# SamArgt/AudioSourceSep

Hardware: NVIDIA B200
Metric: glow_log_prob_samples_per_s (higher is better)
Workload: dtype bf16

## Files before the change

audiosourcesep_b200/csrc/nn_tc.cu:

```cuda
#include "nn_tc_shared.cuh"

namespace asep {

namespace {

constexpr int kBarBytes4 = 256;
constexpr int kSmemBytes4 = kARegionBytes + kStages * kStageBytes + kBiasBytes + kBarBytes4;

template <bool kBwd, bool kSaveMask, bool kF16>
__global__ void __launch_bounds__(kThreadsTC2, 1) k_nn_tc4(const TCParams prm) {
  extern __shared__ __align__(1024) uint8_t smem[];
  if ((smem_u32(smem) & 1023u) != 0u) __trap();
  constexpr int S = kStages;
  uint8_t* sA = smem;
  uint8_t* sB = smem + kARegionBytes;
  float* sBias = reinterpret_cast<float*>(smem + kARegionBytes + S * kStageBytes);
  uint64_t* bars = reinterpret_cast<uint64_t*>(smem + kARegionBytes + S * kStageBytes + kBiasBytes);
  const uint32_t full0 = smem_u32(&bars[0]), empty0 = smem_u32(&bars[S]);
  const uint32_t a1_ready = smem_u32(&bars[2 * S]), accfull0 = smem_u32(&bars[2 * S + 1]);
  const uint32_t accfree_h0 = smem_u32(&bars[2 * S + 3]), panel0 = smem_u32(&bars[2 * S + 4]);
  const uint32_t cons0 = smem_u32(&bars[2 * S + 12]);
  uint32_t* tmem_slot = reinterpret_cast<uint32_t*>(&bars[2 * S + 16]);

  const int warp = threadIdx.x >> 5, lane = threadIdx.x & 31;
  if (threadIdx.x == 0) {
    for (int i = 0; i < S; ++i) {
      mbar_init(full0 + 8 * i, 1);
      mbar_init(empty0 + 8 * i, 1);
    }
    mbar_init(a1_ready, 8);
    mbar_init(accfull0, 1);
    mbar_init(accfull0 + 8, 1);
    mbar_init(accfree_h0, 8);
    for (int i = 0; i < 8; ++i) mbar_init(panel0 + 8 * i, 8);
    for (int i = 0; i < 4; ++i) mbar_init(cons0 + 8 * i, 1);
    fence_barrier_init();
  }
  if (warp == 2) tmem_alloc(smem_u32(tmem_slot), kTmemCols);
  tc_fence_before();
  __syncthreads();
  tc_fence_after();
  const uint32_t tmem_base = *tmem_slot;
  const uint32_t img3_bytes = (uint32_t)prm.n3p * 128u;

  if (warp == 0) {
    if (lane == 0) {
      uint32_t stage = 0, phase = 0;
      const uint8_t* w1 = reinterpret_cast<const uint8_t*>(prm.wimg);
      const uint8_t* w2 = w1 + (size_t)2 * prm.k1_panels * kStageBytes;
      const uint8_t* w3 = w2 + (size_t)2 * kNumPanels * kStageBytes;
      auto push = [&](const uint8_t* src, uint32_t bytes) {
        mbar_wait(empty0 + 8 * stage, phase ^ 1);
        mbar_expect_tx(full0 + 8 * stage, bytes);
        bulk_g2s(smem_u32(sB + stage * kStageBytes), src, bytes, full0 + 8 * stage);
        if (++stage == (uint32_t)S) { stage = 0; phase ^= 1; }
      };
      for (int round = 0; round < prm.num_rounds; ++round) {
        for (int half = 1; half >= 0; --half)
          for (int kp = 0; kp < prm.k1_panels; ++kp) push(w1 + (size_t)(half * prm.k1_panels + kp) * kStageBytes, kStageBytes);
        for (int i = 0; i < 2 * kNumPanels; ++i) push(w2 + (size_t)i * kStageBytes, kStageBytes);
        for (int kp = 0; kp < kNumPanels; ++kp) push(w3 + (size_t)kp * img3_bytes, img3_bytes);
      }
    }
  } else if (warp == 1) {
    if (lane == 0) {
      uint32_t stage = 0, phase = 0;
      const uint32_t a_base = smem_u32(sA);
      constexpr uint32_t idesc256 = make_idesc(256);
      constexpr uint32_t idesc256h = kF16 ? make_idesc_f16(256) : make_idesc(256);
      const uint32_t idesc3 = kF16 ? make_idesc_f16(prm.n3p) : make_idesc(prm.n3p);
      auto kblock = [&](uint32_t d_tmem, int kp, int steps, uint32_t idesc, bool first) {
        mbar_wait(full0 + 8 * stage, phase);
        tc_fence_after();
        const uint64_t da = make_desc(a_base + kp * kPanelBytes);
        const uint64_t db = make_desc(smem_u32(sB + stage * kStageBytes));
        for (int k = 0; k < steps; ++k) umma_bf16(d_tmem, da + (uint64_t)(2 * k), db + (uint64_t)(2 * k), idesc, !(first && k == 0));
        umma_commit(empty0 + 8 * stage);
        if (++stage == (uint32_t)S) { stage = 0; phase ^= 1; }
      };
      const uint32_t h0 = tmem_base, h1 = tmem_base + 256u;
      for (int round = 0; round < prm.num_rounds; ++round) {
        mbar_wait(a1_ready, round & 1);
        tc_fence_after();
        for (int kp = 0; kp < prm.k1_panels; ++kp) kblock(h1, kp, min(4, prm.k1_steps - 4 * kp), idesc256, kp == 0);
        umma_commit(accfull0 + 8);
        if (round > 0) {
          mbar_wait(accfree_h0, (round - 1) & 1);
          tc_fence_after();
        }
        for (int kp = 0; kp < prm.k1_panels; ++kp) kblock(h0, kp, min(4, prm.k1_steps - 4 * kp), idesc256, kp == 0);
        umma_commit(accfull0);
        for (int p = 0; p < 4; ++p) mbar_wait(panel0 + 8 * p, 0);
        tc_fence_after();
        for (int kp = 0; kp < kNumPanels; ++kp) {
          if (kp >= 4) {
            mbar_wait(panel0 + 8 * kp, 0);
            tc_fence_after();
          }
          kblock(h0, kp, 4, idesc256h, kp == 0);
        }
        umma_commit(accfull0);
        for (int kp = 0; kp < kNumPanels; ++kp) {
          kblock(h1, kp, 4, idesc256h, kp == 0);
          if (kp < 4) umma_commit(cons0 + 8 * kp);
        }
        umma_commit(accfull0 + 8);
        for (int p = 0; p < 4; ++p) mbar_wait(panel0 + 8 * p, 1);
        tc_fence_after();
        for (int kp = 0; kp < kNumPanels; ++kp) {
          if (kp >= 4) {
            mbar_wait(panel0 + 8 * kp, 1);
            tc_fence_after();
          }
          kblock(h0, kp, 4, idesc3, kp == 0);
        }
        umma_commit(accfull0);
      }
    }
  } else {
    const int lq = warp & 3;
    const int ch = (warp - 2) >> 2;
    const int row = lq * 32 + lane;
    const int wtid = threadIdx.x - 64;
    const uint32_t t_lane = tmem_base + ((uint32_t)(lq * 32) << 16);
    uint8_t* stg = sA + kARegionBytes - ((kTileM * prm.n3p * 4 + 1023) & ~1023);
    const int k1_pad = prm.k1_steps * 16;
    float4 b1v = make_float4(0.f, 0.f, 0.f, 0.f), b2v = b1v;
    if constexpr (!kBwd) {
      if (wtid < kF / 4) {
        b1v = __ldg(reinterpret_cast<const float4*>(prm.bias1) + wtid);
        b2v = __ldg(reinterpret_cast<const float4*>(prm.bias2) + wtid);
        reinterpret_cast<float4*>(sBias)[wtid] = b1v;
      }
    }
    auto arrive_warp = [&](uint32_t bar) {
      __syncwarp();
      if (lane == 0) mbar_arrive(bar);
    };
    const int tb = ch == 0 ? 0 : 5, te = ch == 0 ? 5 : 9;
    auto row_coords = [&](int round, long long& p, bool& valid, int& h, int& w) {
      const long long tile = (long long)round * prm.tiles_per_cta_round + blockIdx.x;
      p = tile * kTileM + row;
      valid = p < prm.M;
      w = 0; h = 0;
      if (valid) {
        const uint32_t pu = (uint32_t)p, q = pu / (uint32_t)prm.W;
        w = (int)(pu - q * (uint32_t)prm.W);
        h = (int)(q % (uint32_t)prm.H);
      }
    };
    auto finish_a1 = [&]() {
      if (ch == 1)
        for (int k = 2 * 9 * prm.src_ch; k < k1_pad; k += 2)
          *reinterpret_cast<uint32_t*>(sA + a_offset(row, k)) = 0u;
      fence_proxy_async();
      arrive_warp(a1_ready);
    };
    auto build = [&](int round) {
      long long p; bool valid; int h, w;
      row_coords(round, p, valid, h, w);
      build_a1_taps<16>(sA, row, prm.src, p, valid, h, w, prm.H, prm.W, prm.src_stride, prm.src_off, prm.tap_sign, tb, te);
      finish_a1();
    };
    const bool prefetch_regs = prm.src_ch <= 8;
    float pre[40];
    auto prefetch_a1 = [&](int round) {
      long long p; bool valid; int h, w;
      row_coords(round, p, valid, h, w);
      switch (prm.src_ch) {
        case 1: a1_load<1>(pre, prm.src, p, valid, h, w, prm.H, prm.W, prm.src_stride, prm.src_off, prm.tap_sign, tb, te); break;
        case 2: a1_load<2>(pre, prm.src, p, valid, h, w, prm.H, prm.W, prm.src_stride, prm.src_off, prm.tap_sign, tb, te); break;
        case 8: a1_load<8>(pre, prm.src, p, valid, h, w, prm.H, prm.W, prm.src_stride, prm.src_off, prm.tap_sign, tb, te); break;
        default: a1_load<4>(pre, prm.src, p, valid, h, w, prm.H, prm.W, prm.src_stride, prm.src_off, prm.tap_sign, tb, te); break;
      }
    };
    auto store_a1 = [&]() {
      switch (prm.src_ch) {
        case 1: a1_store<1>(sA, row, pre, tb, te); break;
        case 2: a1_store<2>(sA, row, pre, tb, te); break;
        case 8: a1_store<8>(sA, row, pre, tb, te); break;
        default: a1_store<4>(sA, row, pre, tb, te); break;
      }
      finish_a1();
    };
    for (int round = 0; round < prm.num_rounds; ++round) {
      const long long tile = (long long)round * prm.tiles_per_cta_round + blockIdx.x;
      const long long p = tile * kTileM + row;
      const bool valid = p < prm.M;
      const bool stamp = prm.dbg_out != nullptr && blockIdx.x == 0 && wtid == 0;
      long long* ts = prm.dbg_out + (long long)round * 8;
      if (prefetch_regs) {
        if (round == 0) { prefetch_a1(0); store_a1(); }
      } else {
        build(round);
      }
      if (stamp) ts[0] = clock64();
      if (ch == 0) {
        const long long pn = p + 2ll * prm.tiles_per_cta_round * kTileM;
        if (pn < prm.M) asm volatile("prefetch.global.L2 [%0];" ::"l"(prm.src + pn * prm.src_stride));
      }
#pragma unroll 1
      for (int gemm = 0; gemm < 2; ++gemm) {
        uint32_t* mask = kBwd ? (gemm == 0 ? prm.mask2 : prm.mask1) : (gemm == 0 ? prm.mask1 : prm.mask2);
        __nv_bfloat16* dump = gemm == 0 ? prm.dump1 : prm.dump2;
        uint32_t mkl[4] = {0u, 0u, 0u, 0u}, mkh[4] = {0u, 0u, 0u, 0u};
        if constexpr (kBwd) {
          if (valid) {
            const uint4 m0 = __ldg(reinterpret_cast<const uint4*>(mask + p * (kF / 32) + ch * 8));
            const uint4 m1 = __ldg(reinterpret_cast<const uint4*>(mask + p * (kF / 32) + ch * 8) + 1);
            mkl[0] = m0.x; mkl[1] = m0.y; mkl[2] = m0.z; mkl[3] = m0.w; mkh[0] = m1.x; mkh[1] = m1.y; mkh[2] = m1.z; mkh[3] = m1.w;
          }
        }
        if (gemm == 0 && wtid == 0) bulk_wait_read_all();
        if (!kBwd || gemm == 0) named_bar_sync(1, kWorkers2);
#pragma unroll 1
        for (int hh = 0; hh < 2; ++hh) {
          const uint32_t par = hh == 0 ? (uint32_t)(round + gemm) & 1u : (uint32_t)gemm;
          mbar_wait(accfull0 + 8 * hh, par);
          tc_fence_after();
          uint32_t v[2][32];
          tmem_ld32(t_lane + (uint32_t)(hh * 256 + ch * 32), v[0]);
#pragma unroll
          for (int pp = 0; pp < 4; ++pp) {
            const int pn = 4 * hh + pp;
            const int j = 2 * pn + ch;
            tmem_ld_wait();
            if (pp + 1 < 4) tmem_ld32(t_lane + (uint32_t)(hh * 256 + (pp + 1) * 64 + ch * 32), v[(pp + 1) & 1]);
            uint32_t pk[16];
            if constexpr (!kBwd) {
              uint32_t bits = 0;
#pragma unroll
              for (int c4 = 0; c4 < 8; ++c4) {
                const float4 b4 = reinterpret_cast<const float4*>(sBias + j * 32)[c4];
                const float f0 = __uint_as_float(v[pp & 1][4 * c4 + 0]) + b4.x, f1 = __uint_as_float(v[pp & 1][4 * c4 + 1]) + b4.y;
                const float f2 = __uint_as_float(v[pp & 1][4 * c4 + 2]) + b4.z, f3 = __uint_as_float(v[pp & 1][4 * c4 + 3]) + b4.w;
                if constexpr (kSaveMask) {
                  bits |= (f0 > 0.f ? 1u : 0u) << (4 * c4) | (f1 > 0.f ? 1u : 0u) << (4 * c4 + 1) |
                          (f2 > 0.f ? 1u : 0u) << (4 * c4 + 2) | (f3 > 0.f ? 1u : 0u) << (4 * c4 + 3);
                }
                pk[2 * c4] = kF16 ? pack_relu_f16(f0, f1) : pack_relu_bf16(f0, f1);
                pk[2 * c4 + 1] = kF16 ? pack_relu_f16(f2, f3) : pack_relu_bf16(f2, f3);
              }
              if constexpr (kSaveMask) { if (hh) mkh[pp] = bits; else mkl[pp] = bits; }
            } else {
              const uint32_t bits = hh ? mkh[pp] : mkl[pp];
#pragma unroll
              for (int c2 = 0; c2 < 16; ++c2) {
                const float f0 = ((bits >> (2 * c2)) & 1u) ? __uint_as_float(v[pp & 1][2 * c2]) : 0.f;
                const float f1 = ((bits >> (2 * c2 + 1)) & 1u) ? __uint_as_float(v[pp & 1][2 * c2 + 1]) : 0.f;
                pk[c2] = pack_bf16(f0, f1);
              }
            }
            if (dump != nullptr && valid) {
#pragma unroll
              for (int c4 = 0; c4 < 4; ++c4) {
                uint32_t d[4];
#pragma unroll
                for (int q = 0; q < 4; ++q) {
                  if constexpr (!kF16) {
                    d[q] = pk[4 * c4 + q];
                  } else {
                    const float2 f = __half22float2(*reinterpret_cast<const __half2*>(&pk[4 * c4 + q]));
                    d[q] = pack_bf16(f.x, f.y);
                  }
                }
                *reinterpret_cast<uint4*>(dump + p * kF + j * 32 + c4 * 8) = make_uint4(d[0], d[1], d[2], d[3]);
              }
            }
            if (gemm == 1 && hh == 0) mbar_wait(cons0 + 8 * pn, round & 1);
            uint8_t* base = sA + pn * kPanelBytes + row * 128;
#pragma unroll
            for (int c4 = 0; c4 < 4; ++c4)
              *reinterpret_cast<uint4*>(base + (((ch * 4 + c4) ^ (row & 7)) << 4)) =
                  make_uint4(pk[4 * c4], pk[4 * c4 + 1], pk[4 * c4 + 2], pk[4 * c4 + 3]);
            if (hh == 0 ? pp == 3 : (pp & 1)) {
              fence_proxy_async();
              tc_fence_before();
              __syncwarp();
              if (lane == 0) {
                if (hh == 0) {
#pragma unroll
                  for (int q = 0; q < 4; ++q) mbar_arrive(panel0 + 8 * q);
                } else {
                  mbar_arrive(panel0 + 8 * (pn - 1));
                  mbar_arrive(panel0 + 8 * pn);
                }
              }
            }
          }
          if (gemm == 1 && hh == 0 && prefetch_regs && round + 1 < prm.num_rounds) prefetch_a1(round + 1);
        }
        if constexpr (kSaveMask) {
          if (valid) {
            uint4* mo = reinterpret_cast<uint4*>(mask + p * (kF / 32) + ch * 8);
            mo[0] = make_uint4(mkl[0], mkl[1], mkl[2], mkl[3]);
            mo[1] = make_uint4(mkh[0], mkh[1], mkh[2], mkh[3]);
          }
        }
        if constexpr (!kBwd) {
          named_bar_sync(1, kWorkers2);
          if (wtid < kF / 4) reinterpret_cast<float4*>(sBias)[wtid] = gemm == 0 ? b2v : b1v;
        }
        if (stamp) ts[1 + gemm] = clock64();
      }

      mbar_wait(accfull0, (uint32_t)(round + 2) & 1u);
      tc_fence_after();
      if (stamp) ts[3] = clock64();
      if (prefetch_regs && round + 1 < prm.num_rounds) store_a1();
      if (stamp) ts[4] = clock64();
      {
        uint8_t* stg_row = stg + (size_t)row * 16;
        for (int j = ch; j < prm.n3p / 16; j += 4) {
          uint32_t v[2][16];
          const bool two = j + 2 < prm.n3p / 16;
          tmem_ld16(t_lane + (uint32_t)(j * 16), v[0]);
          if (two) tmem_ld16(t_lane + (uint32_t)((j + 2) * 16), v[1]);
          tmem_ld_wait();
#pragma unroll
          for (int i = 0; i < 2; ++i) {
            if (i == 1 && !two) break;
#pragma unroll
            for (int c4 = 0; c4 < 4; ++c4)
              *reinterpret_cast<uint4*>(stg_row + (size_t)((j + 2 * i) * 4 + c4) * (kTileM * 16)) =
                  make_uint4(v[i][4 * c4], v[i][4 * c4 + 1], v[i][4 * c4 + 2], v[i][4 * c4 + 3]);
          }
        }
        tc_fence_before();
        arrive_warp(accfree_h0);
        fence_proxy_async();
        named_bar_sync(2, kWorkers2);
        if (wtid == 0) {
          if (tile * kTileM < prm.M)
            bulk_s2g(prm.out + tile * kTileM * prm.n3p, smem_u32(stg), (uint32_t)(kTileM * prm.n3p * 4));
        }
      }
      if (stamp) ts[5] = clock64();
    }
    if (wtid == 0) bulk_wait_all();
  }

  tc_fence_before();
  __syncthreads();
  if (warp == 2) tmem_dealloc(tmem_base, kTmemCols);
}

int g_num_sms = 0;

bool g_prof_on = false;
std::vector<TcProfToken> g_prof_recs, g_prof_pool;
double g_prof_flops = 0.0;
double g_next_flops = 0.0;


template <bool kBwd, bool kSaveMask, bool kF16>
void launch_tc4(const TCParams& prm, int grid, cudaStream_t s) {
  auto kern = k_nn_tc4<kBwd, kSaveMask, kF16>;
  static bool attr_set = false;
  if (!attr_set) {
    CUDA_CHECK(cudaFuncSetAttribute(kern, cudaFuncAttributeMaxDynamicSharedMemorySize, kSmemBytes4));
    attr_set = true;
  }
  const TcProfToken tok = nn_tc_prof_begin(s);
  kern<<<grid, kThreadsTC2, kSmemBytes4, s>>>(prm);
  ASEP_LAUNCH_CHECK();
  nn_tc_prof_end(tok, s, g_next_flops);
}

template <bool kBwd>
bool run_tc(TCParams prm, cudaStream_t s) {
  if (g_num_sms == 0) {
    int dev = 0;
    CUDA_CHECK(cudaGetDevice(&dev));
    CUDA_CHECK(cudaDeviceGetAttribute(&g_num_sms, cudaDevAttrMultiProcessorCount, dev));
  }
  {
    ASEP_CHECK(prm.k1_panels * kPanelBytes + ((kTileM * prm.n3p * 4 + 1023) & ~1023) <= kARegionBytes, ASEP_ERR_UNSUPPORTED,
               "coupling network shape outside the tcgen05 kernel (stage-1 panels %d, stage-3 columns %d)", prm.k1_panels, prm.n3p);
    ASEP_CHECK(prm.M < (1ll << 31), ASEP_ERR_UNSUPPORTED, "more than 2^31 pixels in one coupling-network launch");
    const long long tiles = (prm.M + kTileM - 1) / kTileM;
    const int grid = (int)std::min<long long>(tiles, g_num_sms);
    prm.tiles_per_cta_round = grid;
    prm.num_rounds = (int)((tiles + grid - 1) / grid);
    static long long* dbg = nullptr;
    static const bool timing = getenv("ASEP_TC_DBG_TIMING") != nullptr;
    if (timing) {
      if (!dbg) CUDA_CHECK(cudaMalloc(&dbg, 8 * 4096 * sizeof(long long)));
      ASEP_CHECK(prm.num_rounds <= 4096, ASEP_ERR_BAD_ARG, "too many rounds for the timing buffer");
      prm.dbg_out = dbg;
    }
    if constexpr (kBwd) {
      launch_tc4<true, false, false>(prm, grid, s);
    } else {
      const bool save = prm.mask1 != nullptr;
      if (prm.f16) { if (save) launch_tc4<false, true, true>(prm, grid, s); else launch_tc4<false, false, true>(prm, grid, s); }
      else { if (save) launch_tc4<false, true, false>(prm, grid, s); else launch_tc4<false, false, false>(prm, grid, s); }
    }
    if (timing) {
      CUDA_CHECK(cudaStreamSynchronize(s));
      std::vector<long long> h((size_t)8 * prm.num_rounds);
      CUDA_CHECK(cudaMemcpy(h.data(), dbg, h.size() * sizeof(long long), cudaMemcpyDeviceToHost));
      double d[6] = {0};
      const int r0 = prm.num_rounds > 2 ? 1 : 0, r1 = prm.num_rounds;
      for (int r = r0; r < r1; ++r) {
        for (int i = 0; i < 5; ++i) d[i] += (double)(h[r * 8 + i + 1] - h[r * 8 + i]);
        if (r + 1 < r1) d[5] += (double)(h[(r + 1) * 8] - h[r * 8 + 5]);
      }
      const double n = r1 - r0;
      fprintf(stderr, "[tc4 %s M=%lld rounds=%d] cycles/tile: S1+E1 %.0f | E2 %.0f | wait S3 %.0f | store next a1 %.0f | E3 %.0f | gap %.0f | total %.0f\n",
              kBwd ? "bwd" : "fwd", prm.M, prm.num_rounds, d[0] / n, d[1] / n, d[2] / n, d[3] / n, d[4] / n,
              d[5] / std::max(1.0, n - 1), (double)(h[(r1 - 1) * 8 + 5] - h[r0 * 8]) / n);
      double ld = 0;
      for (int r = r0; r < r1; ++r) ld += (double)(h[r * 8 + 6] - h[r * 8 + 3]);
      fprintf(stderr, "      first E3 TMEM load complete %.0f cycles after the S3 commit was seen\n", ld / n);
    }
    return true;
  }
}

}

TcProfToken nn_tc_prof_begin(cudaStream_t s) {
  TcProfToken rec{};
  if (!g_prof_on) return rec;
  if (!g_prof_pool.empty()) { rec = g_prof_pool.back(); g_prof_pool.pop_back(); }
  else { CUDA_CHECK(cudaEventCreate(&rec.a)); CUDA_CHECK(cudaEventCreate(&rec.b)); }
  rec.on = true;
  CUDA_CHECK(cudaEventRecord(rec.a, s));
  return rec;
}
void nn_tc_prof_end(const TcProfToken& rec, cudaStream_t s, double flops) {
  if (!rec.on) return;
  CUDA_CHECK(cudaEventRecord(rec.b, s));
  g_prof_recs.push_back(rec);
  g_prof_flops += flops;
}

void nn_tc_profile(int on) {
  g_prof_on = on != 0;
  if (g_prof_on) {
    for (auto& r : g_prof_recs) g_prof_pool.push_back(r);
    g_prof_recs.clear();
    g_prof_flops = 0.0;
  }
}
bool nn_tc_profile_enabled() { return g_prof_on; }
void nn_tc_profile_read(double* total_ms, long long* launches, double* flops) {
  double ms = 0.0;
  for (auto& r : g_prof_recs) {
    CUDA_CHECK(cudaEventSynchronize(r.b));
    float t = 0.f;
    CUDA_CHECK(cudaEventElapsedTime(&t, r.a, r.b));
    ms += t;
  }
  if (total_ms) *total_ms = ms;
  if (launches) *launches = (long long)g_prof_recs.size();
  if (flops) *flops = g_prof_flops;
}

GatherSrc nn_tc_gather_src(const NNWeightsTC& w, const NNScratchTC& sc, bool backward, long long M, int H, int W, bool split) {
  GatherSrc g;
  g.G = sc.G;
  g.const3 = backward ? nullptr : w.const3;
  g.c3 = backward ? nullptr : w.c3;
  g.n3p = backward ? w.bwd.n3p : w.fwd.n3p;
  g.H = H; g.W = W;
  g.nparts = split ? 2 : 1;
  g.part_stride = split ? (M + kTileM - 1) / kTileM * kTileM * (long long)g.n3p : 0;
  return g;
}

size_t nn_tc_g_floats(long long M, int C) { return (size_t)((M + kTileM - 1) / kTileM * kTileM) * (size_t)pad16(9 * C); }

void nn_tc_prepare(NNWeightsTC& w, const float* k1, const float* c1, const float* g1, const float* b1,
                   const float* k2, const float* c2, const float* g2, const float* b2, const float* k3,
                   const float* c3, int C, int F, bool f16, bool x3) {
  ASEP_CHECK(F == kF, ASEP_ERR_UNSUPPORTED, "the tcgen05 coupling kernel is built for n_filters = %d (got %d)", kF, F);
  nn_tc_release(w);
  const int Ch = C / 2;
  {
    const int K1h = 9 * Ch;
    auto f1 = [&](int n, int k) { return k1[(size_t)(k % K1h) * F + n]; };
    auto f2 = [&](int n, int k) { return g1[k] * k2[(size_t)k * F + n]; };
    auto f3 = [&](int n, int k) {
      const int tap = n / C, c = n % C;
      return g2[k] * k3[((size_t)tap * F + k) * C + c];
    };
    const float ws = (f16 && x3) ? 256.f : 1.f;
    build_stage_set(w.fwd, 2 * K1h, 9 * C, f1, f2, f3,  f16,  f16 && x3, false, ws);
    if (x3) build_stage_set(w.fwd_lo, 2 * K1h, 9 * C, f1, f2, f3, f16, f16,  true, ws);
    w.wscale_fwd = ws;
  }
  {
    const int K1h = 9 * C;
    auto f1 = [&](int n, int k) {
      const int kk = k % K1h, tap = kk / C, c = kk % C;
      return g2[n] * k3[((size_t)tap * F + n) * C + c];
    };
    auto f2 = [&](int n, int k) { return g1[n] * k2[(size_t)n * F + k]; };
    auto f3 = [&](int n, int k) { return k1[(size_t)n * F + k]; };
    build_stage_set(w.bwd, 2 * K1h, 9 * Ch, f1, f2, f3, false);
    if (x3) build_stage_set(w.bwd_lo, 2 * K1h, 9 * Ch, f1, f2, f3, false, false,  true);
  }
  std::vector<float> bias1(c1, c1 + F), bias2(F), const3((size_t)9 * C), vc3(c3, c3 + C);
  for (int n = 0; n < F; ++n) {
    double a = c2[n];
    for (int k = 0; k < F; ++k) a += (double)b1[k] * (double)k2[(size_t)k * F + n];
    bias2[n] = (float)a;
  }
  for (int tap = 0; tap < 9; ++tap)
    for (int c = 0; c < C; ++c) {
      double a = 0.0;
      for (int k = 0; k < F; ++k) a += (double)b2[k] * (double)k3[((size_t)tap * F + k) * C + c];
      const3[(size_t)tap * C + c] = (float)a;
    }
  w.bias1 = upload(bias1);
  w.bias2 = upload(bias2);
  w.const3 = upload(const3);
  w.c3 = upload(vc3);
  w.f16 = f16;
  w.x3 = x3;
}

void nn_tc_release(NNWeightsTC& w) {
  if (w.fwd.img) cudaFree(w.fwd.img);
  if (w.bwd.img) cudaFree(w.bwd.img);
  if (w.fwd_lo.img) cudaFree(w.fwd_lo.img);
  if (w.bwd_lo.img) cudaFree(w.bwd_lo.img);
  if (w.bias1) cudaFree(w.bias1);
  if (w.bias2) cudaFree(w.bias2);
  if (w.const3) cudaFree(w.const3);
  if (w.c3) cudaFree(w.c3);
  w = NNWeightsTC{};
}

void nn_tc_forward(const NNWeightsTC& w, const NNScratchTC& sc, const float* state, float* r, uint32_t* mask1,
                   uint32_t* mask2, int N, int H, int W, int C, cudaStream_t s, __nv_bfloat16* dump1,
                   __nv_bfloat16* dump2) {
  const long long M = (long long)N * H * W;
  if (M == 0) return;
  TCParams prm{};
  prm.src = state; prm.src_stride = C; prm.src_off = C / 2; prm.src_ch = C / 2; prm.tap_sign = 1;
  prm.wimg = w.fwd.img; prm.k1_steps = w.fwd.k1_steps; prm.k1_panels = w.fwd.k1_panels; prm.n3p = w.fwd.n3p;
  prm.bias1 = w.bias1; prm.bias2 = w.bias2; prm.mask1 = mask1; prm.mask2 = mask2;
  prm.dump1 = dump1; prm.dump2 = dump2; prm.f16 = w.f16 ? 1 : 0;
  prm.out = sc.G; prm.H = H; prm.W = W; prm.M = M;
  g_next_flops = 2.0 * (double)M * (9.0 * (C / 2) * kF + (double)kF * kF + 9.0 * kF * C);
  run_tc<false>(prm, s);
  if (r != nullptr) launch_gather_fwd(sc.G, w.const3, w.c3, r, M, H, W, C, w.fwd.n3p, 1, 0, s);
}

void nn_tc_backward(const NNWeightsTC& w, const NNScratchTC& sc, const float* gr, const uint32_t* mask1,
                    const uint32_t* mask2, float* gxb, int N, int H, int W, int C, cudaStream_t s,
                    __nv_bfloat16* dump_gp2, __nv_bfloat16* dump_gp1) {
  const long long M = (long long)N * H * W;
  if (M == 0) return;
  TCParams prm{};
  prm.src = gr; prm.src_stride = C; prm.src_off = 0; prm.src_ch = C; prm.tap_sign = -1;
  prm.wimg = w.bwd.img; prm.k1_steps = w.bwd.k1_steps; prm.k1_panels = w.bwd.k1_panels; prm.n3p = w.bwd.n3p;
  prm.bias1 = nullptr; prm.bias2 = nullptr;
  prm.mask1 = const_cast<uint32_t*>(mask1); prm.mask2 = const_cast<uint32_t*>(mask2);
  prm.dump1 = dump_gp2; prm.dump2 = dump_gp1;
  prm.out = sc.G; prm.H = H; prm.W = W; prm.M = M;
  g_next_flops = 2.0 * (double)M * (9.0 * (C / 2) * kF + (double)kF * kF + 9.0 * kF * C);
  run_tc<true>(prm, s);
  if (gxb != nullptr) launch_gather_bwd(sc.G, gxb, M, H, W, C / 2, w.bwd.n3p, 1, 0, s);
}

}
```

Baseline: 18720.

## Ping-pong TMEM accumulators across rounds and split stage-3 MMA chains

The two 256-column TMEM accumulator halves now alternate roles each round, so stage 1 of a round writes into the half freed earliest and the MMA thread waits on accfree only before the second half. The stage-1 A panels move to the tail of the A region and the stage-3 staging buffer moves to the front, with workers waiting on the second accumulator before overwriting panels that alias stage-1 operands. When n3p is small, stage 3 alternates its K steps between two TMEM column ranges to break the serial accumulate dependency, and the epilogue sums both partial results. More detailed MMA-thread wait timing is added behind the debug flag.

```diff
diff --git a/audiosourcesep_b200/csrc/nn_tc.cu b/audiosourcesep_b200/csrc/nn_tc.cu
--- a/audiosourcesep_b200/csrc/nn_tc.cu
+++ b/audiosourcesep_b200/csrc/nn_tc.cu
@@ -18,7 +18,7 @@
   uint64_t* bars = reinterpret_cast<uint64_t*>(smem + kARegionBytes + S * kStageBytes + kBiasBytes);
   const uint32_t full0 = smem_u32(&bars[0]), empty0 = smem_u32(&bars[S]);
   const uint32_t a1_ready = smem_u32(&bars[2 * S]), accfull0 = smem_u32(&bars[2 * S + 1]);
-  const uint32_t accfree_h0 = smem_u32(&bars[2 * S + 3]), panel0 = smem_u32(&bars[2 * S + 4]);
+  const uint32_t accfree = smem_u32(&bars[2 * S + 3]), panel0 = smem_u32(&bars[2 * S + 4]);
   const uint32_t cons0 = smem_u32(&bars[2 * S + 12]);
   uint32_t* tmem_slot = reinterpret_cast<uint32_t*>(&bars[2 * S + 16]);
 
@@ -31,7 +31,7 @@
     mbar_init(a1_ready, 8);
     mbar_init(accfull0, 1);
     mbar_init(accfull0 + 8, 1);
-    mbar_init(accfree_h0, 8);
+    mbar_init(accfree, 8);
     for (int i = 0; i < 8; ++i) mbar_init(panel0 + 8 * i, 8);
     for (int i = 0; i < 4; ++i) mbar_init(cons0 + 8 * i, 1);
     fence_barrier_init();
@@ -42,6 +42,7 @@
   tc_fence_after();
   const uint32_t tmem_base = *tmem_slot;
   const uint32_t img3_bytes = (uint32_t)prm.n3p * 128u;
+  const int a1_panel0 = kNumPanels - prm.k1_panels;
 
   if (warp == 0) {
     if (lane == 0) {
@@ -56,7 +57,7 @@
         if (++stage == (uint32_t)S) { stage = 0; phase ^= 1; }
       };
       for (int round = 0; round < prm.num_rounds; ++round) {
-        for (int half = 1; half >= 0; --half)
+        for (int half = 0; half < 2; ++half)
           for (int kp = 0; kp < prm.k1_panels; ++kp) push(w1 + (size_t)(half * prm.k1_panels + kp) * kStageBytes, kStageBytes);
         for (int i = 0; i < 2 * kNumPanels; ++i) push(w2 + (size_t)i * kStageBytes, kStageBytes);
         for (int kp = 0; kp < kNumPanels; ++kp) push(w3 + (size_t)kp * img3_bytes, img3_bytes);
@@ -69,52 +70,73 @@
       constexpr uint32_t idesc256 = make_idesc(256);
       constexpr uint32_t idesc256h = kF16 ? make_idesc_f16(256) : make_idesc(256);
       const uint32_t idesc3 = kF16 ? make_idesc_f16(prm.n3p) : make_idesc(prm.n3p);
-      auto kblock = [&](uint32_t d_tmem, int kp, int steps, uint32_t idesc, bool first) {
-        mbar_wait(full0 + 8 * stage, phase);
+      const bool split3 = 2 * prm.n3p <= 256;
+      const bool stamp = prm.dbg_out != nullptr && blockIdx.x == 0;
+      long long w_a1 = 0, w_free = 0, w_p2 = 0, w_p3 = 0, w_ring = 0, w_late = 0;
+      auto twait = [&](uint32_t bar, uint32_t par, long long& acc) {
+        if (stamp) {
+          const long long t0 = clock64();
+          mbar_wait(bar, par);
+          acc += clock64() - t0;
+        } else {
+          mbar_wait(bar, par);
+        }
+      };
+      auto kblock = [&](uint32_t d_tmem, int kp, int steps, uint32_t idesc, bool first, uint32_t d_odd) {
+        twait(full0 + 8 * stage, phase, w_ring);
         tc_fence_after();
         const uint64_t da = make_desc(a_base + kp * kPanelBytes);
         const uint64_t db = make_desc(smem_u32(sB + stage * kStageBytes));
-        for (int k = 0; k < steps; ++k) umma_bf16(d_tmem, da + (uint64_t)(2 * k), db + (uint64_t)(2 * k), idesc, !(first && k == 0));
+        const int fresh = d_odd == d_tmem ? 1 : 2;
+        for (int k = 0; k < steps; ++k)
+          umma_bf16((k & 1) ? d_odd : d_tmem, da + (uint64_t)(2 * k), db + (uint64_t)(2 * k), idesc, !(first && k < fresh));
         umma_commit(empty0 + 8 * stage);
         if (++stage == (uint32_t)S) { stage = 0; phase ^= 1; }
       };
-      const uint32_t h0 = tmem_base, h1 = tmem_base + 256u;
       for (int round = 0; round < prm.num_rounds; ++round) {
-        mbar_wait(a1_ready, round & 1);
+        long long* ts = prm.dbg_out + (long long)round * 16;
+        w_a1 = w_free = w_p2 = w_p3 = w_ring = w_late = 0;
+        const uint32_t a = (uint32_t)round & 1u;
+        const uint32_t r0 = tmem_base + 256u * a, r1 = tmem_base + 256u * (a ^ 1u);
+        twait(a1_ready, round & 1, w_a1);
         tc_fence_after();
-        for (int kp = 0; kp < prm.k1_panels; ++kp) kblock(h1, kp, min(4, prm.k1_steps - 4 * kp), idesc256, kp == 0);
+        for (int kp = 0; kp < prm.k1_panels; ++kp) kblock(r0, a1_panel0 + kp, min(4, prm.k1_steps - 4 * kp), idesc256, kp == 0, r0);
+        umma_commit(accfull0);
+        if (round > 0) {
+          twait(accfree, (round - 1) & 1, w_free);
+          tc_fence_after();
+        }
+        for (int kp = 0; kp < prm.k1_panels; ++kp) kblock(r1, a1_panel0 + kp, min(4, prm.k1_steps - 4 * kp), idesc256, kp == 0, r1);
         umma_commit(accfull0 + 8);
-        if (round > 0) {
-          mbar_wait(accfree_h0, (round - 1) & 1);
-          tc_fence_after();
-        }
-        for (int kp = 0; kp < prm.k1_panels; ++kp) kblock(h0, kp, min(4, prm.k1_steps - 4 * kp), idesc256, kp == 0);
-        umma_commit(accfull0);
-        for (int p = 0; p < 4; ++p) mbar_wait(panel0 + 8 * p, 0);
+        for (int p = 0; p < 4; ++p) twait(panel0 + 8 * p, 0, w_p2);
         tc_fence_after();
         for (int kp = 0; kp < kNumPanels; ++kp) {
           if (kp >= 4) {
-            mbar_wait(panel0 + 8 * kp, 0);
+            twait(panel0 + 8 * kp, 0, w_late);
             tc_fence_after();
           }
-          kblock(h0, kp, 4, idesc256h, kp == 0);
+          kblock(r0, kp, 4, idesc256h, kp == 0, r0);
         }
         umma_commit(accfull0);
         for (int kp = 0; kp < kNumPanels; ++kp) {
-          kblock(h1, kp, 4, idesc256h, kp == 0);
+          kblock(r1, kp, 4, idesc256h, kp == 0, r1);
           if (kp < 4) umma_commit(cons0 + 8 * kp);
         }
         umma_commit(accfull0 + 8);
-        for (int p = 0; p < 4; ++p) mbar_wait(panel0 + 8 * p, 1);
+        for (int p = 0; p < 4; ++p) twait(panel0 + 8 * p, 1, w_p3);
         tc_fence_after();
+        if (stamp) ts[12] = clock64();
         for (int kp = 0; kp < kNumPanels; ++kp) {
           if (kp >= 4) {
-            mbar_wait(panel0 + 8 * kp, 1);
+            twait(panel0 + 8 * kp, 1, w_late);
             tc_fence_after();
           }
-          kblock(h0, kp, 4, idesc3, kp == 0);
+          kblock(r0, kp, 4, idesc3, kp == 0, split3 ? r0 + (uint32_t)prm.n3p : r0);
         }
         umma_commit(accfull0);
+        if (stamp) {
+          ts[8] = w_a1; ts[9] = w_free; ts[10] = w_p2; ts[11] = w_p3; ts[13] = w_ring; ts[14] = w_late;
+        }
       }
     }
   } else {
@@ -123,7 +145,8 @@
     const int row = lq * 32 + lane;
     const int wtid = threadIdx.x - 64;
     const uint32_t t_lane = tmem_base + ((uint32_t)(lq * 32) << 16);
-    uint8_t* stg = sA + kARegionBytes - ((kTileM * prm.n3p * 4 + 1023) & ~1023);
+    uint8_t* stg = sA;
+    auto sA1 = [&]() { return sA + (kNumPanels - prm.k1_panels) * kPanelBytes; };
     const int k1_pad = prm.k1_steps * 16;
     float4 b1v = make_float4(0.f, 0.f, 0.f, 0.f), b2v = b1v;
     if constexpr (!kBwd) {
@@ -152,14 +175,14 @@
     auto finish_a1 = [&]() {
       if (ch == 1)
         for (int k = 2 * 9 * prm.src_ch; k < k1_pad; k += 2)
-          *reinterpret_cast<uint32_t*>(sA + a_offset(row, k)) = 0u;
+          *reinterpret_cast<uint32_t*>(sA1() + a_offset(row, k)) = 0u;
       fence_proxy_async();
       arrive_warp(a1_ready);
     };
     auto build = [&](int round) {
       long long p; bool valid; int h, w;
       row_coords(round, p, valid, h, w);
-      build_a1_taps<16>(sA, row, prm.src, p, valid, h, w, prm.H, prm.W, prm.src_stride, prm.src_off, prm.tap_sign, tb, te);
+      build_a1_taps<16>(sA1(), row, prm.src, p, valid, h, w, prm.H, prm.W, prm.src_stride, prm.src_off, prm.tap_sign, tb, te);
       finish_a1();
     };
     const bool prefetch_regs = prm.src_ch <= 8;
@@ -176,10 +199,10 @@
     };
     auto store_a1 = [&]() {
       switch (prm.src_ch) {
-        case 1: a1_store<1>(sA, row, pre, tb, te); break;
-        case 2: a1_store<2>(sA, row, pre, tb, te); break;
-        case 8: a1_store<8>(sA, row, pre, tb, te); break;
-        default: a1_store<4>(sA, row, pre, tb, te); break;
+        case 1: a1_store<1>(sA1(), row, pre, tb, te); break;
+        case 2: a1_store<2>(sA1(), row, pre, tb, te); break;
+        case 8: a1_store<8>(sA1(), row, pre, tb, te); break;
+        default: a1_store<4>(sA1(), row, pre, tb, te); break;
       }
       finish_a1();
     };
@@ -187,8 +210,9 @@
       const long long tile = (long long)round * prm.tiles_per_cta_round + blockIdx.x;
       const long long p = tile * kTileM + row;
       const bool valid = p < prm.M;
+      const uint32_t t_r0 = t_lane | ((uint32_t)(round & 1) << 8);
       const bool stamp = prm.dbg_out != nullptr && blockIdx.x == 0 && wtid == 0;
-      long long* ts = prm.dbg_out + (long long)round * 8;
+      long long* ts = prm.dbg_out + (long long)round * 16;
       if (prefetch_regs) {
         if (round == 0) { prefetch_a1(0); store_a1(); }
       } else {
@@ -216,16 +240,17 @@
 #pragma unroll 1
         for (int hh = 0; hh < 2; ++hh) {
           const uint32_t par = hh == 0 ? (uint32_t)(round + gemm) & 1u : (uint32_t)gemm;
+          const uint32_t t_half = t_r0 ^ ((uint32_t)hh << 8);
           mbar_wait(accfull0 + 8 * hh, par);
           tc_fence_after();
           uint32_t v[2][32];
-          tmem_ld32(t_lane + (uint32_t)(hh * 256 + ch * 32), v[0]);
+          tmem_ld32(t_half + (uint32_t)(ch * 32), v[0]);
 #pragma unroll
           for (int pp = 0; pp < 4; ++pp) {
             const int pn = 4 * hh + pp;
             const int j = 2 * pn + ch;
             tmem_ld_wait();
-            if (pp + 1 < 4) tmem_ld32(t_lane + (uint32_t)(hh * 256 + (pp + 1) * 64 + ch * 32), v[(pp + 1) & 1]);
+            if (pp + 1 < 4) tmem_ld32(t_half + (uint32_t)((pp + 1) * 64 + ch * 32), v[(pp + 1) & 1]);
             uint32_t pk[16];
             if constexpr (!kBwd) {
               uint32_t bits = 0;
@@ -267,6 +292,7 @@
                 *reinterpret_cast<uint4*>(dump + p * kF + j * 32 + c4 * 8) = make_uint4(d[0], d[1], d[2], d[3]);
               }
             }
+            if (gemm == 0 && hh == 0 && pn + prm.k1_panels >= kNumPanels) mbar_wait(accfull0 + 8, 0);
             if (gemm == 1 && hh == 0) mbar_wait(cons0 + 8 * pn, round & 1);
             uint8_t* base = sA + pn * kPanelBytes + row * 128;
 #pragma unroll
@@ -311,23 +337,41 @@
       if (stamp) ts[4] = clock64();
       {
         uint8_t* stg_row = stg + (size_t)row * 16;
-        for (int j = ch; j < prm.n3p / 16; j += 4) {
-          uint32_t v[2][16];
-          const bool two = j + 2 < prm.n3p / 16;
-          tmem_ld16(t_lane + (uint32_t)(j * 16), v[0]);
-          if (two) tmem_ld16(t_lane + (uint32_t)((j + 2) * 16), v[1]);
-          tmem_ld_wait();
-#pragma unroll
-          for (int i = 0; i < 2; ++i) {
-            if (i == 1 && !two) break;
-#pragma unroll
-            for (int c4 = 0; c4 < 4; ++c4)
-              *reinterpret_cast<uint4*>(stg_row + (size_t)((j + 2 * i) * 4 + c4) * (kTileM * 16)) =
-                  make_uint4(v[i][4 * c4], v[i][4 * c4 + 1], v[i][4 * c4 + 2], v[i][4 * c4 + 3]);
+        if (2 * prm.n3p <= 256) {
+          for (int j = ch; j < prm.n3p / 16; j += 2) {
+            uint32_t v[2][16];
+            tmem_ld16(t_r0 + (uint32_t)(j * 16), v[0]);
+            tmem_ld16(t_r0 + (uint32_t)(prm.n3p + j * 16), v[1]);
+            tmem_ld_wait();
+#pragma unroll
+            for (int c4 = 0; c4 < 4; ++c4) {
+              float4 f;
+              f.x = __uint_as_float(v[0][4 * c4]) + __uint_as_float(v[1][4 * c4]);
+              f.y = __uint_as_float(v[0][4 * c4 + 1]) + __uint_as_float(v[1][4 * c4 + 1]);
+              f.z = __uint_as_float(v[0][4 * c4 + 2]) + __uint_as_float(v[1][4 * c4 + 2]);
+              f.w = __uint_as_float(v[0][4 * c4 + 3]) + __uint_as_float(v[1][4 * c4 + 3]);
+              *reinterpret_cast<float4*>(stg_row + (size_t)(j * 4 + c4) * (kTileM * 16)) = f;
+            }
           }
+        } else {
+          for (int j = ch; j < prm.n3p / 16; j += 4) {
+            uint32_t v[2][16];
+            const bool two = j + 2 < prm.n3p / 16;
+            tmem_ld16(t_r0 + (uint32_t)(j * 16), v[0]);
+            if (two) tmem_ld16(t_r0 + (uint32_t)((j + 2) * 16), v[1]);
+            tmem_ld_wait();
+#pragma unroll
+            for (int i = 0; i < 2; ++i) {
+              if (i == 1 && !two) break;
+#pragma unroll
+              for (int c4 = 0; c4 < 4; ++c4)
+                *reinterpret_cast<uint4*>(stg_row + (size_t)((j + 2 * i) * 4 + c4) * (kTileM * 16)) =
+                    make_uint4(v[i][4 * c4], v[i][4 * c4 + 1], v[i][4 * c4 + 2], v[i][4 * c4 + 3]);
+            }
+          }
         }
         tc_fence_before();
-        arrive_warp(accfree_h0);
+        arrive_warp(accfree);
         fence_proxy_async();
         named_bar_sync(2, kWorkers2);
         if (wtid == 0) {
@@ -385,7 +429,7 @@
     static long long* dbg = nullptr;
     static const bool timing = getenv("ASEP_TC_DBG_TIMING") != nullptr;
     if (timing) {
-      if (!dbg) CUDA_CHECK(cudaMalloc(&dbg, 8 * 4096 * sizeof(long long)));
+      if (!dbg) CUDA_CHECK(cudaMalloc(&dbg, 16 * 4096 * sizeof(long long)));
       ASEP_CHECK(prm.num_rounds <= 4096, ASEP_ERR_BAD_ARG, "too many rounds for the timing buffer");
       prm.dbg_out = dbg;
     }
@@ -398,21 +442,24 @@
     }
     if (timing) {
       CUDA_CHECK(cudaStreamSynchronize(s));
-      std::vector<long long> h((size_t)8 * prm.num_rounds);
+      std::vector<long long> h((size_t)16 * prm.num_rounds);
       CUDA_CHECK(cudaMemcpy(h.data(), dbg, h.size() * sizeof(long long), cudaMemcpyDeviceToHost));
-      double d[6] = {0};
+      double d[6] = {0}, m[7] = {0};
       const int r0 = prm.num_rounds > 2 ? 1 : 0, r1 = prm.num_rounds;
       for (int r = r0; r < r1; ++r) {
-        for (int i = 0; i < 5; ++i) d[i] += (double)(h[r * 8 + i + 1] - h[r * 8 + i]);
-        if (r + 1 < r1) d[5] += (double)(h[(r + 1) * 8] - h[r * 8 + 5]);
+        const long long* t = &h[(size_t)r * 16];
+        for (int i = 0; i < 5; ++i) d[i] += (double)(t[i + 1] - t[i]);
+        if (r + 1 < r1) d[5] += (double)(t[16] - t[5]);
+        m[0] += t[8]; m[1] += t[9]; m[2] += t[10]; m[3] += t[11]; m[4] += t[14]; m[5] += t[13];
+        m[6] += (double)(t[3] - t[12]);
       }
       const double n = r1 - r0;
       fprintf(stderr, "[tc4 %s M=%lld rounds=%d] cycles/tile: S1+E1 %.0f | E2 %.0f | wait S3 %.0f | store next a1 %.0f | E3 %.0f | gap %.0f | total %.0f\n",
               kBwd ? "bwd" : "fwd", prm.M, prm.num_rounds, d[0] / n, d[1] / n, d[2] / n, d[3] / n, d[4] / n,
-              d[5] / std::max(1.0, n - 1), (double)(h[(r1 - 1) * 8 + 5] - h[r0 * 8]) / n);
-      double ld = 0;
-      for (int r = r0; r < r1; ++r) ld += (double)(h[r * 8 + 6] - h[r * 8 + 3]);
-      fprintf(stderr, "      first E3 TMEM load complete %.0f cycles after the S3 commit was seen\n", ld / n);
+              d[5] / std::max(1.0, n - 1), (double)(h[(size_t)(r1 - 1) * 16 + 5] - h[(size_t)r0 * 16]) / n);
+      fprintf(stderr, "      mma thread waits/tile: a1_ready %.0f | accfree %.0f | first 4 panels S2 %.0f | first 4 panels S3 %.0f | "
+              "later panels %.0f | weight ring %.0f | S3 issue -> S3 complete seen by workers %.0f\n",
+              m[0] / n, m[1] / n, m[2] / n, m[3] / n, m[4] / n, m[5] / n, m[6] / n);
     }
     return true;
   }
```

Result: no change. 18560 (median of 6 runs) (-0.9%).
